# deevinandu/Distributed-Multi-Agent-SLAM-Swarm-Robotics-System

Measured on AMD Instinct MI355X. Metric: QuasarPackets/sec into 4096^2 grid, higher is better.
Workload: dtype f64

## Files before the change

### distributed-multi-agent-slam-swarm-robotics-system_amd/_lib.py

```python
import ctypes as C
import os
import subprocess

_HERE = os.path.dirname(os.path.abspath(__file__))
CSRC = os.path.join(_HERE, "csrc")
LIB_PATH = os.environ.get("QUASAR_SLAM_LIB") or os.path.join(CSRC, "libquasar_slam.so")
HEADER = os.path.join(os.path.dirname(_HERE), "include", "quasar_slam.h")

QS_CNT_NAMES = ("datagrams", "accepted", "rays", "cells", "hits", "closures", "landmarks", "rebases",
                "slam_windows", "slam_rounds", "slam_node_iters", "slam_misc_iters", "slam_cycles",
                "slam_realtime_100mhz", "slam_cyc_prepare", "slam_cyc_query", "slam_cyc_commit", "ekf_wrap_clamp", "edge_rays", "edge_overflow")
QS_FT_MAX_BOTS = 1024
QS_STAGE_NAMES = ("decode", "slam", "raycast", "ekf", "slam_chain", "rc_rays", "rc_sort", "rc_raster")
UINT64_MAX = (1 << 64) - 1
QS_PLAN_STATUS = ("ok", "no_start", "no_goal", "unreachable")


class QsPlanParams(C.Structure):
    _fields_ = [("clearance", C.c_int32), ("snap_radius", C.c_int32), ("lookahead", C.c_int32), ("reserved", C.c_int32)]


class QsGainParams(C.Structure):
    _fields_ = [("range", C.c_int32), ("bias", C.c_uint32), ("reserved", C.c_int32 * 2)]

# ... 141 lines not shown
    "qs_sense_ranges": (_i32, [_vp, _vp, _sz, _i32, _vp, _vp, _vp]),
    "qs_sense_ranges_device": (_i32, [_vp, _vp, _sz, _i32, _vp, _vp, _vp]),
    "qs_sense_sweeps": (_i32, [_vp, _vp, _vp, _vp, _vp, _sz, _vp, _vp, _sz]),
    "qs_sense_sweeps_device": (_i32, [_vp, _vp, _vp, _vp, _vp, _sz, _vp, _vp, _sz]),
    "qs_sense_packets": (_i32, [_vp, _vp, _vp, _vp, _vp, _vp, _sz, _vp, _vp]),
    "qs_sense_packets_device": (_i32, [_vp, _vp, _vp, _vp, _vp, _vp, _sz, _vp, _vp]),
    "qs_last_hits": (_i32, [_vp, _vp, _vp, _sz]),
    "qs_update_rays": (_i32, [_vp, _vp, _vp, _vp, _vp, _vp, _sz, _u64]),
    "qs_world_to_grid": (_i32, [_vp, _vp, _sz, _i32, _vp]),
    "qs_grid_i8": (_i32, [_vp, _vp]),
    "qs_grid_i8_device": (_i32, [_vp, _vp]),
    "qs_grid_counts": (_i32, [_vp, _vp, _vp]),
    "qs_grid_logodds": (_i32, [_vp, _f32, _f32, _f32, _f32, _vp]),
    "qs_device_buffers": (_i32, [_vp, C.POINTER(_vp), C.POINTER(_sz), C.POINTER(_vp), C.POINTER(_sz)]),
    "qs_slam_sizes": (_i32, [_vp, _i32, C.POINTER(_i64), C.POINTER(_i64), C.POINTER(_i64)]),
    "qs_slam_closures": (_i32, [_vp, _i32, _vp, _vp, _sz]),
    "qs_slam_closure_agents": (_i32, [_vp, _i32, _vp, _sz]),
    "qs_slam_landmarks": (_i32, [_vp, _i32, _vp, _vp, _sz]),
    "qs_slam_add_poses": (_i32, [_vp, _vp, _vp, _vp, _vp, _sz, _vp, _vp]),
    "qs_drift": (_i32, [_vp, _i32, _vp]),
    "qs_zone": (_i32, [_vp, _i32, _vp, C.POINTER(_i32)]),
    "qs_zone_packet": (_i32, [_vp, _i32, _i32, _vp]),
    "qs_fuse": (_i32, [_vp, C.POINTER(_vp), _sz]),
    "qs_fuse_buffers": (_i32, [_vp, C.POINTER(_vp), C.POINTER(_vp), _sz]),
    "qs_fuse_buffers_range": (_i32, [_vp, C.POINTER(_vp), C.POINTER(_vp), _sz, _sz, _sz, _i32]),
    "qs_fused_counts": (_i32, [_vp, C.POINTER(_vp), C.POINTER(_sz)]),
    "qs_counts_source": (_i32, [_vp, _i32]),
    "qs_epoch_query": (_i32, [_vp, _u64, _sz, C.POINTER(_i32)]),
    "qs_mark_fused": (_i32, [_vp]),
    "qs_dirty_tracking": (_i32, [_vp, _i32]),
    "qs_dirty_blocks": (_i32, [_vp, C.POINTER(_sz), C.POINTER(_sz)]),
    "qs_sparse_fuse_begin": (_i32, [_vp, _i32, _i32, C.POINTER(_vp), C.POINTER(_sz)]),
    "qs_sparse_fuse_plan": (_i32, [_vp, _vp, _vp, C.POINTER(_vp), C.POINTER(_sz)]),
    "qs_sparse_fuse_apply": (_i32, [_vp]),
    "qs_fused_counts_buffer": (_i32, [_vp, C.POINTER(_vp), C.POINTER(_sz)]),
    "qs_rccl_unique_id": (_i32, [_vp]),
    "qs_rccl_comm_init": (_i32, [_vp, _vp, _i32, _i32, C.POINTER(_vp)]),
    "qs_rccl_comm_destroy": (_i32, [_vp]),
    "qs_sparse_fuse_rccl": (_i32, [_vp, _vp, _i32, _i32, _vp]),
    "qs_grid_to_pcd": (_i32, [_vp, _vp, _i32, _i32, _f64, _f64, _f64, _vp, _sz, C.POINTER(_sz)]),
    "qs_rasterise": (_i32, [_vp, _vp, _sz, _f64, _vp, _vp, _vp]),
    "qs_icp": (_i32, [_vp, _vp, _sz, _vp, _sz, _f64, _i32, _f64, _f64, _vp, _vp, _vp, _vp]),
    "qs_nn_search": (_i32, [_vp, _vp, _sz, _vp, _sz, _f64, _i32, _vp, _vp, _vp]),
    "qs_diag_mfma_f64_rate": (_i32, [_vp, C.POINTER(_f64)]),
    "qs_diag_latencies": (_i32, [_vp, _vp]),
    "qs_set_chain_form": (_i32, [_vp, _i32]),
    "qs_chain_form": (_i32, [_vp]),
    "qs_set_chain_lean": (_i32, [_vp, _i32, _i64]),
    "qs_chain_lean": (_i32, [_vp]),
    "qs_set_chain_lookahead": (_i32, [_vp, _i32]),
    "qs_chain_lookahead": (_i32, [_vp]),
    "qs_set_chain_plan": (_i32, [_vp, _i32]),
    "qs_chain_plan": (_i32, [_vp]),
    "qs_voxel_downsample": (_i32, [_vp, _vp, _sz, _f64, _vp, _sz, C.POINTER(_sz)]),
    "qs_voxel_downsample_device": (_i32, [_vp, _vp, _sz, _f64, _vp, _sz, C.POINTER(_sz)]),
    "qs_merge_reset": (_i32, [_vp]),
    "qs_merge_params": (_i32, [_vp, _f64, _i32, _f64]),
    "qs_merge_grid": (_i32, [_vp, _vp, _i32, _i32, _f64, _f64, _f64, _vp]),
    "qs_merge_grid_device": (_i32, [_vp, _vp, _i32, _i32, _f64, _f64, _f64, _vp]),
    "qs_merge_map": (_i32, [_vp, _vp, _vp]),
    "qs_merge_cloud": (_i32, [_vp, _vp, _sz, C.POINTER(_sz)]),
    "qs_merge_global_map": (_i32, [_vp, _vp, _vp, _vp]),
    "qs_frontier_cells": (_i32, [_vp, _vp, _sz, C.POINTER(_sz)]),
    "qs_frontier_members": (_i32, [_vp, _vp, _sz, C.POINTER(_sz)]),
    "qs_frontier_clusters": (_i32, [_vp, _i32, _vp, _sz, C.POINTER(_sz)]),
    "qs_frontier_targets": (_i32, [_vp, _i32, _f64, _vp, _sz, _vp, _vp, _vp, _sz, C.POINTER(_sz), _vp]),
    "qs_traversable": (_i32, [_vp, _i32, _vp]),
    "qs_plan_field": (_i32, [_vp, _vp, _vp, _vp]),
    "qs_plan_paths": (_i32, [_vp, _vp, _vp, _vp, _sz, _vp, _vp, _vp, _vp, _vp, _sz, _vp, _vp]),
    "qs_frontier_targets_by_path": (_i32, [_vp, _i32, _f64, _vp, _vp, _sz, _vp, _vp, _vp, _vp, _vp, _vp, _vp, _sz,
                                           C.POINTER(_sz), _vp]),
    "qs_frontier_gain": (_i32, [_vp, _i32, _i32, _vp, _vp, _sz, C.POINTER(_sz)]),
    "qs_frontier_targets_by_gain": (_i32, [_vp, _i32, _f64, _vp, _vp, _vp, _sz, _vp, _vp, _vp, _vp, _vp, _vp, _vp, _sz,
                                           C.POINTER(_sz), _vp, _vp]),
    "qs_territories": (_i32, [_vp, _vp, _vp, _sz, _vp, _vp, _vp, _vp, _vp, _vp]),
    "qs_frontier_targets_by_territory": (_i32, [_vp, _i32, _vp, _vp, _sz, _vp, _vp, _vp, _vp, _vp, _vp, _vp, _vp, _vp, _vp, _sz,
                                                C.POINTER(_sz), _vp]),
    "qs_render_view": (_i32, [_vp, _vp, _vp, _sz, _vp, _sz, _vp]),
    "qs_render_view_device": (_i32, [_vp, _vp, _vp, _sz, _vp, _sz, _vp]),
    "qs_ekf_init": (_i32, [_vp, _i32, _f64, _vp]),
    "qs_ekf_step": (_i32, [_vp, _vp, _vp, _vp, _vp, _vp, _sz, _i32]),
    "qs_ekf_state": (_i32, [_vp, _i32, _vp, _vp]),
    "qs_counters": (_i32, [_vp, _vp]),
    "qs_checkpoint": (_i32, [_vp, _vp, _sz, C.POINTER(_sz)]),
    "qs_restore": (_i32, [_vp, _vp, _sz]),
    "qs_timing_enable": (_i32, [_vp, _i32]),
    "qs_stage_times": (_i32, [_vp, _vp, _vp, _i32]),
}


def load():
    global _lib
    if _lib is not None:
        return _lib
    if not os.path.exists(LIB_PATH):
        raise QuasarError(
            f"{LIB_PATH} not found: build it with __graft_entry__.build() (hipcc --offload-arch=gfx950). "
            "There is no CPU fallback for the mapper path.")
    L = C.CDLL(LIB_PATH)
    for name, (res, args) in SIGNATURES.items():
        fn = getattr(L, name)
        fn.restype = res
        fn.argtypes = args
    _lib = L
    return L

# ... 6 lines not shown
```

### distributed-multi-agent-slam-swarm-robotics-system_amd/csrc/qs_api.hip

```cpp
#include <math.h>
#include <algorithm>
#include <mutex>
#include <stdio.h>
#include <stdlib.h>
#include <string.h>

#include "qs_internal.h"
#include "raycast_common.h"

static thread_local std::string g_create_err;

int qs_fail(qs_ctx *c, int code, const char *what, hipError_t e)
{
    char buf[512];
    if (e != hipSuccess) snprintf(buf, sizeof buf, "%s: %s", what, hipGetErrorString(e));
    else snprintf(buf, sizeof buf, "%s", what);
    if (c) c->err = buf; else g_create_err = buf;
    return code;
}

extern "C" const char *qs_version(void) { return "quasar-slam-amd 0.1 (gfx950)"; }

extern "C" int qs_config_default(qs_config *cfg)
{
// ... 280 lines not shown
        HIPCHK(c, hipStreamCreateWithFlags(&c->stream, hipStreamNonBlocking));
        c->own_stream = true;
    }
    return QS_OK;
}

extern "C" int qs_set_chain_form(qs_ctx *c, int form)
{
    ARGCHK(c, c != nullptr);
    ARGCHK(c, form == QS_CHAIN_AUTO || form == QS_CHAIN_FREE || form == QS_CHAIN_WINDOW || form == QS_CHAIN_FREE_POSTING);
    c->chain_form = form;
    return QS_OK;
}

extern "C" int qs_chain_form(qs_ctx *c)
{
    if (!c) return QS_E_INVAL;
    return !c->chain_last_free ? QS_CHAIN_WINDOW : c->chain_last_posting ? QS_CHAIN_FREE_POSTING : QS_CHAIN_FREE;
}

extern "C" int qs_set_chain_lean(qs_ctx *c, int32_t mode, int64_t limit)
{
    ARGCHK(c, c != nullptr);
    ARGCHK(c, mode == QS_CHAIN_LEAN_AUTO || mode == QS_CHAIN_LEAN_OFF);
    c->chain_lean_mode = mode;
    c->chain_lean_limit = limit > 0 && limit < 0x7f7f7f7fll ? limit : 0x7f7f7f7fll;
    return QS_OK;
}

extern "C" int qs_chain_lean(qs_ctx *c)
{
    if (!c) return QS_E_INVAL;
    if (!c->chain_last_lean_asked) return 0;
    unsigned int refused = 0;
    HIPCHK(c, hipMemcpyAsync(&refused, c->d_flags.p + QS_FLAG_CHAIN_FULL, sizeof refused, hipMemcpyDeviceToHost, c->stream));
    HIPCHK(c, hipStreamSynchronize(c->stream));
    return refused != c->chain_lean_seq ? 1 : 0;
}

extern "C" int qs_set_chain_plan(qs_ctx *c, int32_t on)
{
    ARGCHK(c, c != nullptr);
    c->chain_plan = on != 0;
    return QS_OK;
}

extern "C" int qs_chain_plan(qs_ctx *c)
{
    if (!c) return QS_E_INVAL;
    if (!c->chain_last_plan) return 0;
    return qs_chain_lean(c);
}

extern "C" int qs_set_chain_lookahead(qs_ctx *c, int32_t on)
{
    ARGCHK(c, c != nullptr);
    c->chain_lookahead = on != 0;
    return QS_OK;
}

extern "C" int qs_chain_lookahead(qs_ctx *c)
{
    if (!c) return QS_E_INVAL;
    return c->chain_lookahead ? 1 : 0;
}

extern "C" int qs_sync(qs_ctx *c)
{
    ARGCHK(c, c != nullptr);
    HIPCHK(c, hipSetDevice(c->device));
    SYNCCHK(c);
    HIPCHK(c, hipStreamSynchronize(c->stream));
    return QS_OK;
}

extern "C" int qs_reset(qs_ctx *c)
{
    ARGCHK(c, c != nullptr);
    HIPCHK(c, hipSetDevice(c->device));
    return reset_state(c);
}

extern "C" int qs_set_bot_offset(qs_ctx *c, int32_t bot, double off_x)
{
    ARGCHK(c, c != nullptr);
    if (bot < 1 || bot > c->cfg.max_agent) return qs_fail(c, QS_E_RANGE, "qs_set_bot_offset: bot out of range");
    HIPCHK(c, hipSetDevice(c->device));
    HIPCHK(c, hipMemcpyAsync(c->d_offset.p + bot, &off_x, sizeof(double), hipMemcpyHostToDevice, c->stream));
    HIPCHK(c, hipStreamSynchronize(c->stream));
    return QS_OK;
}

extern "C" int qs_timing_enable(qs_ctx *c, int32_t enable)
{
    ARGCHK(c, c != nullptr);
    c->timing = enable != 0;
    return QS_OK;
}

extern "C" int qs_stage_times(qs_ctx *c, double ms[QS_STAGE_N], uint64_t launches[QS_STAGE_N], int32_t reset)
{
    ARGCHK(c, c != nullptr);
    HIPCHK(c, hipSetDevice(c->device));
    HIPCHK(c, hipStreamSynchronize(c->stream));
    for (auto &p : c->pending) {
        float t = 0.f;
// ... 676 lines not shown
```

### distributed-multi-agent-slam-swarm-robotics-system_amd/csrc/slam.hip

```cpp
#include "qs_internal.h"
#include <cstdlib>
#include <cstring>

#define LL_MAX 0x7fffffffffffffffll
#define IDX_BLOCK QS_SLAM_IDX_BLOCK
#define IDX_WAVES (IDX_BLOCK / QS_WAVE)

int qs_slam_blocks(size_t n) { return (int)((n + IDX_BLOCK - 1) / IDX_BLOCK); }

__global__ void __launch_bounds__(IDX_BLOCK)
qs_slam_count_kernel(size_t n, QsBatch b, QsSlamBatch sb, int bots_per_graph, int n_graphs)
{
    __shared__ unsigned int s_acc[QS_MAX_AGENT + 1], s_ev[QS_MAX_AGENT + 1];
    const int tid = threadIdx.x;
    for (int t = tid; t < n_graphs; t += IDX_BLOCK) { s_acc[t] = 0; s_ev[t] = 0; }
    __syncthreads();
    const size_t i = (size_t)blockIdx.x * IDX_BLOCK + tid;
    if (i < n && b.accept[i]) {
        const int g = ((int)b.agent[i] - 1) / bots_per_graph;
        atomicAdd(&s_acc[g], 1u);
        if (b.lm[i]) atomicAdd(&s_ev[g], 1u);
    }
    __syncthreads();
    for (int t = tid; t < n_graphs; t += IDX_BLOCK) {
        sb.blk_acc[(size_t)t * sb.n_blocks + blockIdx.x] = s_acc[t];
        sb.blk_ev[(size_t)t * sb.n_blocks + blockIdx.x] = s_ev[t];
    }
}

__global__ void __launch_bounds__(256)
qs_slam_blockscan_kernel(QsSlamBatch sb)
{
    __shared__ unsigned int s_a[256], s_e[256];
    const int g = blockIdx.x, tid = threadIdx.x;
    unsigned int *acc = sb.blk_acc + (size_t)g * sb.n_blocks, *ev = sb.blk_ev + (size_t)g * sb.n_blocks;
    const int per = (sb.n_blocks + 255) / 256;
    const int lo = min(tid * per, sb.n_blocks), hi = min(lo + per, sb.n_blocks);
    unsigned int a = 0, e = 0;
    for (int k = lo; k < hi; k++) { a += acc[k]; e += ev[k]; }
    s_a[tid] = a; s_e[tid] = e;
    __syncthreads();
    if (tid == 0) {
        unsigned int ra = 0, re = 0;
        for (int t = 0; t < 256; t++) { const unsigned int va = s_a[t], ve = s_e[t]; s_a[t] = ra; s_e[t] = re; ra += va; re += ve; }
        sb.acc_total[g] = ra;
        sb.ev_base[g + 1] = re;
    }
    __syncthreads();
    unsigned int ra = s_a[tid], re = s_e[tid];
    for (int k = lo; k < hi; k++) { const unsigned int va = acc[k], ve = ev[k]; acc[k] = ra; ev[k] = re; ra += va; re += ve; }
}

__global__ void qs_slam_prefix_kernel(QsSlamBatch sb, int n_graphs, int max_agent, const double *__restrict__ drift)
{
    if (threadIdx.x == 0) {
        unsigned int run = 0;
        sb.ev_base[0] = 0;
        for (int g = 0; g < n_graphs; g++) { run += sb.ev_base[g + 1]; sb.ev_base[g + 1] = run; }
    }
    if (threadIdx.x == 64) {
        unsigned int run = 0;
        for (int a = 0; a <= max_agent + 1; a++) { const unsigned int v = a <= max_agent ? sb.agent_ev[a] : 0; sb.agent_ev[a] = run; run += v; }
    }
    for (int t = threadIdx.x; t <= max_agent; t += blockDim.x) {
        sb.acl_cnt[t] = 0;
        sb.drift_start[2 * t] = drift[2 * t];
        sb.drift_start[2 * t + 1] = drift[2 * t + 1];
    }
}

__global__ void __launch_bounds__(IDX_BLOCK)
qs_slam_index_kernel(size_t n, QsBatch b, QsSlamBatch sb, const QsGraphDev *__restrict__ graphs,
                     int bots_per_graph, int n_graphs)
{
    extern __shared__ unsigned int s_w[];
    const int tid = threadIdx.x, lane = tid & 63, wave = tid >> 6;
    for (int t = tid; t < IDX_WAVES * n_graphs * 2; t += IDX_BLOCK) s_w[t] = 0;
    __syncthreads();
    const size_t i = (size_t)blockIdx.x * IDX_BLOCK + tid;
    const bool acc = i < n && b.accept[i];
    int g = -1, agent = 0, lmk = 0;
    if (acc) { agent = b.agent[i]; g = (agent - 1) / bots_per_graph; lmk = b.lm[i]; }
    unsigned int rank = 0, rank_ev = 0;
    unsigned long long remaining = __ballot(acc);
    while (remaining) {
        const int leader = __ffsll((long long)remaining) - 1;
        const int k = __shfl(g, leader);
        const unsigned long long grp = __ballot(acc && g == k);
        const unsigned long long egrp = __ballot(acc && g == k && lmk != 0);
        if (acc && g == k) {
            rank = __popcll(grp & ((1ull << lane) - 1));
            rank_ev = __popcll(egrp & ((1ull << lane) - 1));
            if (lane == leader) {
                s_w[(wave * n_graphs + k) * 2] = __popcll(grp);
                s_w[(wave * n_graphs + k) * 2 + 1] = __popcll(egrp);
            }
        }
        remaining &= ~grp;
    }
    __syncthreads();
    if (acc) {
        unsigned int off = 0, off_ev = 0;
        for (int w = 0; w < wave; w++) { off += s_w[(w * n_graphs + g) * 2]; off_ev += s_w[(w * n_graphs + g) * 2 + 1]; }
        const long long node = graphs[g].n_nodes + sb.blk_acc[(size_t)g * sb.n_blocks + blockIdx.x] + off + rank;
        sb.node[i] = node;
        if (lmk) {
            const size_t e = (size_t)sb.ev_base[g] + sb.blk_ev[(size_t)g * sb.n_blocks + blockIdx.x] + off_ev + rank_ev;
            sb.ev_node[e] = node;
            sb.ev_agent[e] = (unsigned char)(agent - 1 - g * bots_per_graph);
            sb.ev_type[e] = (unsigned char)lmk;
            sb.ev_px[e] = b.px[i];
            sb.ev_py[e] = b.py[i];
        }
    } else if (i < n) {
        sb.node[i] = -1;
    }
}

#define PLAN_BLOCK QS_SLAM_PLAN_BLOCK
#define PLAN_WAVES (PLAN_BLOCK / QS_WAVE)
int qs_slam_plan_blocks(size_t n) { return (int)((n + PLAN_BLOCK - 1) / PLAN_BLOCK); }

__device__ inline int plan_graph_of(const unsigned int *__restrict__ ev_base, int n_graphs, unsigned int e)
{
    int lo = 0, hi = n_graphs - 1;
    while (lo < hi) { const int mid = (lo + hi + 1) >> 1; if (ev_base[mid] <= e) lo = mid; else hi = mid - 1; }
    return lo;
}

__global__ void __launch_bounds__(PLAN_BLOCK)
qs_slam_plan_count_kernel(QsSlamBatch sb, int bots_per_graph, int n_graphs, int max_agent)
{
    __shared__ unsigned int s_cnt[QS_MAX_AGENT + 1];
    const int tid = threadIdx.x;
    const unsigned int n_ev = sb.ev_base[n_graphs], e = blockIdx.x * PLAN_BLOCK + tid;
    if (blockIdx.x * PLAN_BLOCK >= n_ev) return;
    for (int t = tid; t <= max_agent; t += PLAN_BLOCK) s_cnt[t] = 0;
    __syncthreads();
    if (e < n_ev) atomicAdd(&s_cnt[plan_graph_of(sb.ev_base, n_graphs, e) * bots_per_graph + 1 + sb.ev_agent[e]], 1u);
    __syncthreads();
    for (int t = tid; t <= max_agent; t += PLAN_BLOCK) sb.pl_blk[(size_t)t * sb.pl_blocks + blockIdx.x] = s_cnt[t];
}

__global__ void __launch_bounds__(256)
qs_slam_plan_scan_kernel(QsSlamBatch sb, int n_graphs)
{
    __shared__ unsigned int s_c[256];
    const int tid = threadIdx.x;
    const int used = (int)((sb.ev_base[n_graphs] + PLAN_BLOCK - 1) / PLAN_BLOCK);
    unsigned int *cnt = sb.pl_blk + (size_t)blockIdx.x * sb.pl_blocks;
    const int per = (used + 255) / 256;
    const int lo = min(tid * per, used), hi = min(lo + per, used);
    unsigned int c = 0;
    for (int k = lo; k < hi; k++) c += cnt[k];
    s_c[tid] = c;
    __syncthreads();
    for (int d = 1; d < 256; d <<= 1) {
        const unsigned int v = tid >= d ? s_c[tid - d] : 0u;
        __syncthreads();
        s_c[tid] += v;
        __syncthreads();
    }
    unsigned int run = s_c[tid] - c;
    for (int k = lo; k < hi; k++) { const unsigned int v = cnt[k]; cnt[k] = run; run += v; }
}

__global__ void __launch_bounds__(PLAN_BLOCK)
qs_slam_plan_scatter_kernel(QsSlamBatch sb, int bots_per_graph, int n_graphs, int max_agent)
{
    __shared__ unsigned int s_w[PLAN_WAVES][QS_MAX_AGENT + 1];
    const int tid = threadIdx.x, lane = tid & 63, wave = tid >> 6;
    const unsigned int n_ev = sb.ev_base[n_graphs], e = blockIdx.x * PLAN_BLOCK + tid;
    if (blockIdx.x * PLAN_BLOCK >= n_ev) return;
    for (int t = tid; t < PLAN_WAVES * (QS_MAX_AGENT + 1); t += PLAN_BLOCK) (&s_w[0][0])[t] = 0;
    __syncthreads();
    const bool have = e < n_ev;
    int g = 0, bot = -1;
    if (have) { g = plan_graph_of(sb.ev_base, n_graphs, e); bot = g * bots_per_graph + 1 + sb.ev_agent[e]; }
    unsigned int rank = 0;
    unsigned long long remaining = __ballot(have);
    while (remaining) {
        const int k = __shfl(bot, __ffsll((long long)remaining) - 1);
        const unsigned long long grp = __ballot(have && bot == k);
        if (have && bot == k) {
            rank = __popcll(grp & ((1ull << lane) - 1));
            if (rank == 0) s_w[wave][k] = __popcll(grp);
        }
        remaining &= ~grp;
    }
    __syncthreads();
    if (have && bot <= max_agent) {
        unsigned int off = sb.pl_blk[(size_t)bot * sb.pl_blocks + blockIdx.x] + rank;
        for (int w = 0; w < wave; w++) off += s_w[w][bot];
        QsPlanRec rec;
        rec.node = (int)sb.ev_node[e]; rec.r = e - sb.ev_base[g]; rec.type = sb.ev_type[e]; rec.skip = 0;
        rec.px = sb.ev_px[e]; rec.py = sb.ev_py[e];
        sb.pl_rec[sb.agent_ev[bot] + off] = rec;
    }
}

__device__ inline unsigned int plan_first_at_least(const QsPlanRec *pl, unsigned int from, unsigned int n_own, long long bound)
{
    unsigned int lo = from, hi = n_own, step = 1;
    while (lo < n_own) {
        const unsigned int p = step - 1 < n_own - 1 - lo ? lo + step - 1 : n_own - 1;
        if ((long long)pl[p].node >= bound) { hi = p; break; }
        lo = p + 1;
        if (step < (1u << 30)) step <<= 1;
    }
    while (lo < hi) { const unsigned int mid = lo + ((hi - lo) >> 1); if ((long long)pl[mid].node >= bound) hi = mid; else lo = mid + 1; }
    return lo;
}

__global__ void __launch_bounds__(256)
qs_slam_plan_skip_kernel(QsSlamBatch sb, int n_graphs, int max_agent, int min_between, const long long *__restrict__ last_closure)
{
    const unsigned int n_ev = sb.ev_base[n_graphs], s = blockIdx.x * 256 + threadIdx.x;
    if (s >= n_ev) return;
    int lo = 0, hi = max_agent;
    while (lo < hi) { const int mid = (lo + hi + 1) >> 1; if (sb.agent_ev[mid] <= s) lo = mid; else hi = mid - 1; }
    const int bot = lo;
    if (bot < 1) return;
    const unsigned int base = sb.agent_ev[bot], n_own = sb.agent_ev[bot + 1] - base, j = s - base;
    const QsPlanRec *const pl = sb.pl_rec + base;
    sb.pl_rec[base + j].skip = plan_first_at_least(pl, j + 1, n_own, (long long)pl[j].node + (long long)min_between);
    if (j == 0) sb.pl_first[bot] = plan_first_at_least(pl, 0, n_own, last_closure[bot] + (long long)min_between);
}

#define CH_WAVES 16
#define CH_PILE_NODES 64
#define CH_THREADS (CH_WAVES * QS_WAVE)
#define CH_INS (CH_WAVES - 1)
#define CH_FETCH (CH_WAVES - 2)
#define CH_AGW (CH_WAVES - 3)

__device__ inline void lds_barrier()
{
    __builtin_amdgcn_fence(__ATOMIC_RELEASE, "workgroup", "local");
    __builtin_amdgcn_s_barrier();
    __builtin_amdgcn_fence(__ATOMIC_ACQUIRE, "workgroup", "local");
}

__device__ inline int bucket_coord(double v, double b0, double inv_cell)
{
    const double f = floor((v - b0) * inv_cell);
    return (int)fmin(fmax(f, -1.0e9), 1.0e9);
}

__device__ inline long long rl64(long long v, int src_lane)
{
    int lo = (int)(v & 0xffffffffll), hi = (int)(v >> 32);
    lo = __builtin_amdgcn_readlane(lo, src_lane);
    hi = __builtin_amdgcn_readlane(hi, src_lane);
    return ((long long)hi << 32) | (unsigned int)lo;
}

__device__ inline unsigned int bucket_hash(int cx, int cy, unsigned int hmask)
{
    unsigned int h = ((unsigned int)cx * 0x9E3779B1u) ^ ((unsigned int)cy * 0x85EBCA77u);
    h ^= h >> 15;
    return h & hmask;
}
__device__ inline bool bucket_cell(double x, double y, int type, const QsBucketGeom &bg, int &cx, int &cy)
{
    cx = bucket_coord(x, bg.bx0, bg.inv_cell); cy = bucket_coord(y, bg.by0, bg.inv_cell);
    return type >= 1 && type <= QS_NTYPES;
}
__device__ inline long long bucket_key(int type, int cx, int cy, const QsBucketGeom &bg)
{
    return (long long)(type - 1) * ((long long)bg.hmask + 1) + bucket_hash(cx, cy, bg.hmask);
}


#define QS_GLOBAL __attribute__((address_space(1)))
typedef const QS_GLOBAL QsLmNode *QsNodeG;
typedef const QS_GLOBAL unsigned int *QsU32G;

__device__ inline void chain_insert_lanes(const QsGraphDev &G, bool inw, int rank, long long idx, long long kb, double x, double y,
                                          int type, int k, int lane, long long &n_lms, long long &n_misc, unsigned int &pool, bool &pile)
// ... 1212 lines not shown
    auto load = [&](long long e, double &x, double &y, long long &idx, int &type) {
        const bool in = e + lane < L.n;
        x = in ? L.x[e + lane] : 0.0; y = in ? L.y[e + lane] : 0.0;
        idx = in ? L.idx[e + lane] : LL_MAX; type = in ? (int)L.type[e + lane] : 0;
    };
    double x, y; long long idx; int type;
    load(0, x, y, idx, type);
    for (long long e = 0; e < L.n; e += QS_WAVE) {
        double xn, yn; long long idxn; int typen;
        load(e + QS_WAVE, xn, yn, idxn, typen);
        const int k = (int)(L.n - e < QS_WAVE ? L.n - e : QS_WAVE);
        const bool inw = lane < k;
        int cx, cy;
        const long long kb = (inw && bucket_cell(x, y, type, bg, cx, cy)) ? bucket_key(type, cx, cy, bg) : -1;
        chain_insert_lanes(G, inw, lane, idx, kb, x, y, type, k, lane, n_lms, n_misc, pool, pile);
        x = xn; y = yn; idx = idxn; type = typen;
    }
    if (lane == 0) {
        Gp->n_nodes = L.n_nodes; Gp->n_cls = L.n_cls;
        Gp->n_lms = n_lms; Gp->n_misc = n_misc; Gp->nodes_used = pool;
        if (pile) *pile_flag = 1u;
    }
}
hipError_t qs_launch_slam_rebuild_index(qs_ctx *c, const QsIndexLog *d_logs)
{
    if (c->n_graphs <= 0) return hipSuccess;
    hipLaunchKernelGGL(qs_slam_rebuild_index_kernel, dim3(c->n_graphs), dim3(QS_WAVE), 0, c->stream, c->d_graphs.p, c->bg, d_logs,
                       c->d_flags.p + QS_FLAG_PILE);
    return hipGetLastError();
}

hipError_t qs_launch_slam(qs_ctx *c, size_t n, bool raw_pose)
{
    if (n == 0) return hipSuccess;
    QsSlamBatch sb = c->sb;
    sb.n_blocks = qs_slam_blocks(n);
    const int G = c->n_graphs;
    hipLaunchKernelGGL(qs_slam_count_kernel, dim3(sb.n_blocks), dim3(IDX_BLOCK), 0, c->stream, n, c->b, sb,
                       c->bots_per_graph, G);
    hipLaunchKernelGGL(qs_slam_blockscan_kernel, dim3(G), dim3(256), 0, c->stream, sb);
    hipLaunchKernelGGL(qs_slam_prefix_kernel, dim3(1), dim3(256), 0, c->stream, sb, G, c->cfg.max_agent, c->d_drift.p);
    hipLaunchKernelGGL(qs_slam_index_kernel, dim3(sb.n_blocks), dim3(IDX_BLOCK), (size_t)IDX_WAVES * G * 2 * sizeof(unsigned int),
                       c->stream, n, c->b, sb, c->d_graphs.p, c->bots_per_graph, G);
    const bool one = c->bots_per_graph <= CH_AGW;
    const bool free_mode = c->chain_form != QS_CHAIN_WINDOW && !(c->chain_form == QS_CHAIN_AUTO && one && c->chain_windowed);
    const bool post = c->chain_form == QS_CHAIN_FREE_POSTING || (c->chain_form == QS_CHAIN_AUTO && c->chain_posting);
    const int sel = (c->pile_mode ? 4 : 0) | (c->bots_per_graph <= 5 ? 2 : 0) | (post ? 1 : 0);
    const bool lean_asked = free_mode && one && c->chain_lean_mode != QS_CHAIN_LEAN_OFF && !post && sel != 6;
    const bool plan = lean_asked && c->chain_plan && !raw_pose && !c->pile_mode;
    c->chain_last_plan = plan;
    if (plan) {
        sb.pl_blocks = qs_slam_plan_blocks(n);
        const int nbots = c->cfg.max_agent + 1;
        hipLaunchKernelGGL(qs_slam_plan_count_kernel, dim3(sb.pl_blocks), dim3(PLAN_BLOCK), 0, c->stream, sb, c->bots_per_graph, G, c->cfg.max_agent);
        hipLaunchKernelGGL(qs_slam_plan_scan_kernel, dim3(nbots), dim3(256), 0, c->stream, sb, G);
        hipLaunchKernelGGL(qs_slam_plan_scatter_kernel, dim3(sb.pl_blocks), dim3(PLAN_BLOCK), 0, c->stream, sb, c->bots_per_graph, G, c->cfg.max_agent);
        hipLaunchKernelGGL(qs_slam_plan_skip_kernel, dim3((unsigned int)((n + 255) / 256)), dim3(256), 0, c->stream, sb, G,
                           c->cfg.max_agent, c->cfg.min_poses_between, c->d_last_closure.p);
    } else {
        sb.pl_rec = nullptr;
    }
    StageTimer t_chain(c, QS_STAGE_SLAM_CHAIN);
#define CH_LAUNCH(ONE_, DENSE_) hipLaunchKernelGGL((qs_slam_chain_kernel<ONE_, DENSE_>), dim3(G), dim3(CH_THREADS), 0, c->stream, c->d_graphs.p, sb, c->bg, \
                           c->bots_per_graph, c->cfg.max_agent, c->win, c->cfg.min_poses_between, c->r2_threshold,                          \
                           c->cfg.closure_correction, c->d_drift.p, c->d_last_closure.p, c->d_counters.p, raw_pose ? 1 : 0, c->d_flags.p + QS_FLAG_PILE)
    c->chain_last_posting = false;
    c->chain_last_free = free_mode;
    c->chain_last_lean_asked = false;
#define FR_LAUNCH(DENSE_, WAVES_, POST_) hipLaunchKernelGGL((qs_slam_chain_free_kernel<DENSE_, WAVES_, POST_>), dim3(G), dim3(WAVES_ * QS_WAVE), 0, c->stream, c->d_graphs.p, sb, c->bg, \
                           c->bots_per_graph, c->cfg.max_agent, c->cfg.min_poses_between, c->r2_threshold,                                  \
                           c->cfg.closure_correction, c->d_drift.p, c->d_last_closure.p, c->d_counters.p, raw_pose ? 1 : 0, c->d_flags.p + QS_FLAG_PILE, \
                           c->chain_lean_mode == QS_CHAIN_LEAN_OFF ? 0ll : c->chain_lean_limit, c->chain_lean_seq,                          \
                           (unsigned int)((c->chain_lookahead ? QS_NODE_LOOKAHEAD : QS_NODE_CAP - 1) * sizeof(long long)))
#define DY_LAUNCH(DENSE_) hipLaunchKernelGGL((qs_slam_chain_dyn_kernel<DENSE_>), dim3(G), dim3(CH_THREADS), 0, c->stream, c->d_graphs.p, sb, c->bg, \
                           c->bots_per_graph, c->cfg.max_agent, c->cfg.min_poses_between, c->r2_threshold,                                  \
                           c->cfg.closure_correction, c->d_drift.p, c->d_last_closure.p, c->d_counters.p, raw_pose ? 1 : 0, c->d_flags.p + QS_FLAG_PILE)
    if (free_mode) {
        if (one) {
            c->chain_lean_seq++;
            c->chain_last_lean_asked = lean_asked;
            switch (sel) {
            case 0: FR_LAUNCH(false, 16, false); break;  case 1: FR_LAUNCH(false, 16, true); break;
            case 2: FR_LAUNCH(false, 8, false); break;   case 3: FR_LAUNCH(false, 8, true); break;
            case 4: FR_LAUNCH(true, 16, false); break;   case 5: FR_LAUNCH(true, 16, true); break;
            case 6: FR_LAUNCH(true, 8, false); break;    default: FR_LAUNCH(true, 8, true); break;
            }
            c->chain_last_posting = post;
        }
        else { if (c->pile_mode) DY_LAUNCH(true); else DY_LAUNCH(false); }
    }
#undef DY_LAUNCH
    else if (c->pile_mode) { if (one) CH_LAUNCH(true, true); else CH_LAUNCH(false, true); }
    else { if (one) CH_LAUNCH(true, false); else CH_LAUNCH(false, false); }
#undef FR_LAUNCH
#undef CH_LAUNCH
    t_chain.stop();
    if (raw_pose) return hipGetLastError();
    hipLaunchKernelGGL(qs_slam_pose_kernel, dim3((unsigned int)((n + 255) / 256)), dim3(256), 0, c->stream, n, c->b, sb);
    return hipGetLastError();
}
```

### distributed-multi-agent-slam-swarm-robotics-system_amd/mapper.py

```python
import ctypes as C
import os
import struct
import types
import zlib

import numpy as np

from . import _lib
from ._lib import QsConfig, QsMergeResult, QsViewParams, QS_MERGE_STATUS, QuasarError, UINT64_MAX, check
from . import protocol as P


def _ptr(a):
    return a.ctypes.data_as(C.c_void_p) if a is not None else None


def _dev_addr(a):
    return int(a.data_ptr()) if hasattr(a, "data_ptr") else int(a or 0)


CKPT_MAGIC = b"QSCK"
CKPT_VERSION = 1
CKPT_HEADER_FIXED = 144
CKPT_SECTIONS = {1: "scalars", 2: "bots", 3: "counters", 4: "graphs", 5: "block_ids", 6: "blocks", 7: "dirty"}
# ... 749 lines not shown
        dims = np.zeros(2, dtype=np.int32)
        origin = np.zeros(2, dtype=np.float64)
        self._chk(self._L.qs_rasterise(self._h, _ptr(xy), len(xy), res, _ptr(dims), _ptr(origin), None),
                  "qs_rasterise")
        if len(xy) == 0:
            return None, None
        grid = np.empty((int(dims[0]), int(dims[1])), dtype=np.int8)
        self._chk(self._L.qs_rasterise(self._h, _ptr(xy), len(xy), res, _ptr(dims), _ptr(origin), _ptr(grid)),
                  "qs_rasterise")
        return grid, origin

    def icp(self, src_xy, dst_xy, max_dist=1.0, max_iter=30, rel_fitness=1e-6, rel_rmse=1e-6):
        a = np.ascontiguousarray(src_xy, dtype=np.float64); b = np.ascontiguousarray(dst_xy, dtype=np.float64)
        T = np.zeros(9, dtype=np.float64)
        fit, rm, it = C.c_double(), C.c_double(), C.c_int32()
        self._chk(self._L.qs_icp(self._h, _ptr(a), len(a), _ptr(b), len(b), max_dist, max_iter, rel_fitness, rel_rmse,
                                 _ptr(T), C.byref(fit), C.byref(rm), C.byref(it)), "qs_icp")
        return T.reshape(3, 3), fit.value, rm.value, it.value

    def nn_search(self, src_xy, dst_xy, max_dist=1.0, mode=0):
        a = np.ascontiguousarray(src_xy, dtype=np.float64); b = np.ascontiguousarray(dst_xy, dtype=np.float64)
        corr = np.empty(len(a), dtype=np.int32); d2 = np.empty(len(a), dtype=np.float64)
        ms = np.zeros(2, dtype=np.float32)
        self._chk(self._L.qs_nn_search(self._h, _ptr(a), len(a), _ptr(b), len(b), max_dist, mode, _ptr(corr), _ptr(d2), _ptr(ms)),
                  "qs_nn_search")
        return corr, d2, (float(ms[0]), float(ms[1]))

    CHAIN_FORMS = {"auto": 0, "free": 1, "window": 2, "free_posting": 3}

    def set_chain_form(self, form):
        self._chk(self._L.qs_set_chain_form(self._h, self.CHAIN_FORMS[form]), "qs_set_chain_form")

    def chain_form(self):
        return {1: "free", 2: "window", 3: "free_posting"}[self._L.qs_chain_form(self._h)]

    def set_chain_lean(self, mode="auto", limit=0):
        self._chk(self._L.qs_set_chain_lean(self._h, {"auto": 0, "off": 1}[mode], int(limit)), "qs_set_chain_lean")

    def chain_lean(self):
        r = self._L.qs_chain_lean(self._h)
        if r < 0:
            self._chk(r, "qs_chain_lean")
        return bool(r)

    def set_chain_plan(self, on=True):
        self._chk(self._L.qs_set_chain_plan(self._h, 1 if on else 0), "qs_set_chain_plan")

    def chain_plan(self):
        r = self._L.qs_chain_plan(self._h)
        if r < 0:
            self._chk(r, "qs_chain_plan")
        return bool(r)

    def set_chain_lookahead(self, on=True):
        self._chk(self._L.qs_set_chain_lookahead(self._h, 1 if on else 0), "qs_set_chain_lookahead")

    def chain_lookahead(self):
        r = self._L.qs_chain_lookahead(self._h)
        if r < 0:
            self._chk(r, "qs_chain_lookahead")
        return bool(r)

    def mfma_f64_rate(self):
        v = C.c_double()
        self._chk(self._L.qs_diag_mfma_f64_rate(self._h, C.byref(v)), "qs_diag_mfma_f64_rate")
        return v.value

    def diag_latencies(self):
        out = np.zeros(9, dtype=np.float64)
        self._chk(self._L.qs_diag_latencies(self._h, _ptr(out)), "qs_diag_latencies")
        names = ("l2_load", "l1_load", "lds_read", "fma_f64", "dpp_step", "readlane_step", "barrier_16_waves", "barrier_5_waves", "clock_mhz")
        return dict(zip(names, (float(v) for v in out)))

    def voxel_downsample(self, xy, voxel):
        a = np.ascontiguousarray(xy, dtype=np.float64)
        n = C.c_size_t()
        self._chk(self._L.qs_voxel_downsample(self._h, _ptr(a), len(a), voxel, None, 0, C.byref(n)), "qs_voxel_downsample")
        out = np.zeros((n.value, 2), dtype=np.float64)
        if n.value:
            self._chk(self._L.qs_voxel_downsample(self._h, _ptr(a), len(a), voxel, _ptr(out), n.value, C.byref(n)),
                      "qs_voxel_downsample")
        return out

    def voxel_downsample_device(self, d_xy, n, voxel, d_out=0, cap=0):
        k = C.c_size_t()
        self._chk(self._L.qs_voxel_downsample_device(self._h, C.c_void_p(_dev_addr(d_xy)), int(n), voxel,
                                                     C.c_void_p(_dev_addr(d_out)), int(cap), C.byref(k)), "qs_voxel_downsample_device")
        return k.value

    def merge_reset(self):
        self._chk(self._L.qs_merge_reset(self._h), "qs_merge_reset")

    def merge_params(self, icp_threshold=1.0, icp_iterations=30, min_fitness=0.6):
        self._chk(self._L.qs_merge_params(self._h, icp_threshold, icp_iterations, min_fitness), "qs_merge_params")

    @staticmethod
    def _merge_result(r):
        return {"status": QS_MERGE_STATUS[r.status], "iterations": int(r.iterations), "n_local": int(r.n_local),
                "n_global": int(r.n_global), "fitness": float(r.fitness), "rmse": float(r.rmse),
                "T": np.array(r.T, dtype=np.float64).reshape(3, 3)}

    def merge_grid(self, grid, res, ox, oy):
        r = QsMergeResult()
        if hasattr(grid, "data_ptr"):
            if not (grid.is_cuda and grid.is_contiguous() and grid.dim() == 2 and grid.element_size() == 1):
                raise ValueError("merge_grid: a device grid is a contiguous 2-D int8 tensor on the GPU")
# ... 510 lines not shown
```

### include/quasar_slam.h

```cpp
#ifndef QUASAR_SLAM_H
#define QUASAR_SLAM_H

#include <stddef.h>
#include <stdint.h>

#ifdef __cplusplus
extern "C" {
#endif

#define QS_OK 0
#define QS_E_INVAL (-1)
#define QS_E_HIP (-2)
#define QS_E_NOMEM (-3)
#define QS_E_RANGE (-4)
#define QS_E_NODEV (-5)
#define QS_E_STATE (-6)

#define QS_PACKET_SIZE 42
#define QS_PACKET_SIZE_V1 41
#define QS_ZONE_SIZE 20

typedef struct qs_ctx qs_ctx;

typedef struct qs_config {
// ... 133 lines not shown
                      const uint8_t *landmark, size_t n, uint8_t *closed, double *corr2);
int qs_drift(qs_ctx *ctx, int32_t bot, double out[2]);

int qs_zone(qs_ctx *ctx, int32_t bot, double out[4], int32_t *valid);
int qs_zone_packet(qs_ctx *ctx, int32_t bot, int32_t online, uint8_t out[QS_ZONE_SIZE]);

int qs_fuse(qs_ctx *dst, qs_ctx *const *srcs, size_t n);
int qs_fuse_buffers(qs_ctx *dst, const void *const *stamps_dev, const void *const *counts_dev,
                    size_t n);
int qs_fuse_buffers_range(qs_ctx *dst, const void *const *stamps_dev, const void *const *counts_dev,
                          size_t n, size_t cell_offset, size_t n_cells, int32_t counts_into_fused);
int qs_fused_counts(qs_ctx *ctx, void **fused_dev, size_t *bytes);
int qs_counts_source(qs_ctx *ctx, int32_t fused);
int qs_epoch_query(qs_ctx *ctx, uint64_t seq0, size_t n, int32_t *would_rebase);
int qs_mark_fused(qs_ctx *ctx);
#define QS_DIRTY_BLOCK_W 16
#define QS_DIRTY_BLOCK_H 4
#define QS_SPARSE_MAX_WORLD 64
int qs_dirty_tracking(qs_ctx *ctx, int32_t enable);
int qs_dirty_blocks(qs_ctx *ctx, size_t *n_blocks, size_t *block_cells);
int qs_sparse_fuse_begin(qs_ctx *ctx, int32_t world, int32_t rank, void **bitmaps_dev, size_t *bitmap_bytes);
int qs_sparse_fuse_plan(qs_ctx *ctx, uint32_t *n_blocks , size_t *offsets ,
                        void **payload_dev, size_t *block_bytes);
int qs_sparse_fuse_apply(qs_ctx *ctx);
#define QS_RCCL_ID_BYTES 128
int qs_rccl_unique_id(uint8_t out[QS_RCCL_ID_BYTES]);
int qs_rccl_comm_init(qs_ctx *ctx, const uint8_t id[QS_RCCL_ID_BYTES], int32_t world, int32_t rank, void **comm);
int qs_rccl_comm_destroy(void *comm);
int qs_sparse_fuse_rccl(qs_ctx *ctx, void *comm, int32_t world, int32_t rank, uint64_t stats[4]);
int qs_fused_counts_buffer(qs_ctx *ctx, void **fused_dev, size_t *bytes);
int qs_grid_to_pcd(qs_ctx *ctx, const int8_t *grid, int32_t h, int32_t w, double res,
                   double ox, double oy, double *xy, size_t cap, size_t *n_out);
int qs_rasterise(qs_ctx *ctx, const double *xy, size_t n, double res, int32_t dims[2],
                 double origin[2], int8_t *grid);

int qs_icp(qs_ctx *ctx, const double *src_xy, size_t n_src, const double *dst_xy, size_t n_dst,
           double max_dist, int32_t max_iter, double rel_fitness, double rel_rmse, double T[9],
           double *fitness, double *rmse, int32_t *iters);
int qs_nn_search(qs_ctx *ctx, const double *src_xy, size_t n_src, const double *dst_xy, size_t n_dst,
                 double max_dist, int32_t mode, int32_t *corr, double *d2, float ms[2]);
#define QS_CHAIN_AUTO 0
#define QS_CHAIN_FREE 1
#define QS_CHAIN_WINDOW 2
#define QS_CHAIN_FREE_POSTING 3
int qs_set_chain_form(qs_ctx *ctx, int form);
int qs_chain_form(qs_ctx *ctx);
#define QS_CHAIN_LEAN_AUTO 0
#define QS_CHAIN_LEAN_OFF 1
int qs_set_chain_lean(qs_ctx *ctx, int32_t mode, int64_t limit);
int qs_chain_lean(qs_ctx *ctx);

int qs_set_chain_plan(qs_ctx *ctx, int32_t on);
int qs_chain_plan(qs_ctx *ctx);

int qs_set_chain_lookahead(qs_ctx *ctx, int32_t on);
int qs_chain_lookahead(qs_ctx *ctx);

int qs_diag_mfma_f64_rate(qs_ctx *ctx, double *tflops);
#define QS_DIAG_LAT_N 9
int qs_diag_latencies(qs_ctx *ctx, double out[QS_DIAG_LAT_N]);
int qs_voxel_downsample(qs_ctx *ctx, const double *xy, size_t n, double voxel, double *out_xy,
                        size_t cap, size_t *n_out);

int qs_voxel_downsample_device(qs_ctx *ctx, const double *d_xy, size_t n, double voxel, double *d_out_xy,
                               size_t cap, size_t *n_out);

enum { QS_MERGE_EMPTY = 0, QS_MERGE_ADOPTED = 1, QS_MERGE_MERGED = 2, QS_MERGE_REJECTED = 3 };
typedef struct qs_merge_result {
    int32_t status, iterations;
    uint64_t n_local, n_global;
    double fitness, rmse, T[9];
} qs_merge_result;
int qs_merge_reset(qs_ctx *ctx);
int qs_merge_params(qs_ctx *ctx, double icp_threshold, int32_t icp_iterations, double min_fitness);
int qs_merge_grid(qs_ctx *ctx, const int8_t *grid, int32_t h, int32_t w, double res, double ox, double oy,
                  qs_merge_result *out);
int qs_merge_grid_device(qs_ctx *ctx, const int8_t *d_grid, int32_t h, int32_t w, double res, double ox, double oy,
                         qs_merge_result *out);
int qs_merge_map(qs_ctx *ctx, qs_ctx *src, qs_merge_result *out);
int qs_merge_cloud(qs_ctx *ctx, double *xy, size_t cap, size_t *n_out);
int qs_merge_global_map(qs_ctx *ctx, int32_t dims[2], double origin[2], int8_t *grid);

int qs_frontier_cells(qs_ctx *ctx, int32_t *xy, size_t cap, size_t *n_out);
int qs_frontier_clusters(qs_ctx *ctx, int32_t min_cluster, int64_t *stats5, size_t cap, size_t *n_out);

int qs_frontier_members(qs_ctx *ctx, int32_t *xy_root, size_t cap, size_t *n_out);

#define QS_FT_MAX_BOTS 1024
int qs_frontier_targets(qs_ctx *ctx, int32_t min_cluster, double separation,
                        const double *bot_xy, size_t n_bots, int64_t *target_idx, double *target_xy,
                        double *centroids_xy, size_t cap, size_t *n_centroids, uint64_t stats[4]);

#define QS_PLAN_OK 0
#define QS_PLAN_NO_START 1
#define QS_PLAN_NO_GOAL 2
#define QS_PLAN_UNREACHABLE 3
#define QS_PLAN_ORTHO 5
#define QS_PLAN_DIAG 7
#define QS_PLAN_MAX_CLEARANCE 16
#define QS_PLAN_MAX_SNAP 64
#define QS_PLAN_MAX_LOOKAHEAD 65536
#define QS_PLAN_WS_CAP ((size_t)2 << 30)
typedef struct qs_plan_params { int32_t clearance, snap_radius, lookahead, reserved; } qs_plan_params;
int qs_traversable(qs_ctx *ctx, int32_t clearance, uint8_t *mask_host);
int qs_plan_field(qs_ctx *ctx, const qs_plan_params *params, const double goal_xy[2], uint32_t *field_host);
int qs_plan_paths(qs_ctx *ctx, const qs_plan_params *params, const double *start_xy, const double *goal_xy, size_t n,
// ... 107 lines not shown
```

Before: 102.2 million.

## Fold plan skip computation into scatter kernel with shared-memory halo search

```diff
diff --git a/distributed-multi-agent-slam-swarm-robotics-system_amd/_lib.py b/distributed-multi-agent-slam-swarm-robotics-system_amd/_lib.py
--- a/distributed-multi-agent-slam-swarm-robotics-system_amd/_lib.py
+++ b/distributed-multi-agent-slam-swarm-robotics-system_amd/_lib.py
@@ -217,6 +217,7 @@
     "qs_chain_lookahead": (_i32, [_vp]),
     "qs_set_chain_plan": (_i32, [_vp, _i32]),
     "qs_chain_plan": (_i32, [_vp]),
+    "qs_chain_plan_read": (_i32, [_vp, _i32, _vp, _vp, _vp, _sz, C.POINTER(_sz), C.POINTER(C.c_uint32)]),
     "qs_voxel_downsample": (_i32, [_vp, _vp, _sz, _f64, _vp, _sz, C.POINTER(_sz)]),
     "qs_voxel_downsample_device": (_i32, [_vp, _vp, _sz, _f64, _vp, _sz, C.POINTER(_sz)]),
     "qs_merge_reset": (_i32, [_vp]),
diff --git a/distributed-multi-agent-slam-swarm-robotics-system_amd/csrc/qs_api.hip b/distributed-multi-agent-slam-swarm-robotics-system_amd/csrc/qs_api.hip
--- a/distributed-multi-agent-slam-swarm-robotics-system_amd/csrc/qs_api.hip
+++ b/distributed-multi-agent-slam-swarm-robotics-system_amd/csrc/qs_api.hip
@@ -356,6 +356,28 @@
     return qs_chain_lean(c);
 }
 
+extern "C" int qs_chain_plan_read(qs_ctx *c, int32_t bot, int32_t *node, uint32_t *r, uint32_t *skip, size_t cap, size_t *n_own,
+                                  uint32_t *first)
+{
+    ARGCHK(c, c != nullptr && n_own && first);
+    ARGCHK(c, (node && r && skip) || (!node && !r && !skip));
+    if (bot < 1 || bot > c->cfg.max_agent) return qs_fail(c, QS_E_RANGE, "qs_chain_plan_read: bot out of range");
+    if (!c->chain_last_plan) return qs_fail(c, QS_E_STATE, "qs_chain_plan_read: the last ingest had no plan");
+    HIPCHK(c, hipSetDevice(c->device));
+    unsigned int range[2] = {0, 0}, f = 0;
+    HIPCHK(c, hipMemcpyAsync(range, c->sb.agent_ev + bot, sizeof range, hipMemcpyDeviceToHost, c->stream));
+    HIPCHK(c, hipMemcpyAsync(&f, c->sb.pl_first + bot, sizeof f, hipMemcpyDeviceToHost, c->stream));
+    HIPCHK(c, hipStreamSynchronize(c->stream));
+    const size_t n = range[1] - range[0];
+    *n_own = n; *first = f;
+    if (!node) return QS_OK;
+    if (n > cap) return qs_fail(c, QS_E_RANGE, "qs_chain_plan_read: capacity too small");
+    std::vector<QsPlanRec> rec(n);
+    if (n) HIPCHK(c, hipMemcpy(rec.data(), c->sb.pl_rec + range[0], n * sizeof(QsPlanRec), hipMemcpyDeviceToHost));
+    for (size_t i = 0; i < n; i++) { node[i] = rec[i].node; r[i] = rec[i].r; skip[i] = rec[i].skip; }
+    return QS_OK;
+}
+
 extern "C" int qs_set_chain_lookahead(qs_ctx *c, int32_t on)
 {
     ARGCHK(c, c != nullptr);
diff --git a/distributed-multi-agent-slam-swarm-robotics-system_amd/csrc/slam.hip b/distributed-multi-agent-slam-swarm-robotics-system_amd/csrc/slam.hip
--- a/distributed-multi-agent-slam-swarm-robotics-system_amd/csrc/slam.hip
+++ b/distributed-multi-agent-slam-swarm-robotics-system_amd/csrc/slam.hip
@@ -64,6 +64,7 @@
     }
     for (int t = threadIdx.x; t <= max_agent; t += blockDim.x) {
         sb.acl_cnt[t] = 0;
+        sb.pl_first[t] = 0;
         sb.drift_start[2 * t] = drift[2 * t];
         sb.drift_start[2 * t + 1] = drift[2 * t + 1];
     }
@@ -129,17 +130,25 @@
 }
 
 __global__ void __launch_bounds__(PLAN_BLOCK)
-qs_slam_plan_count_kernel(QsSlamBatch sb, int bots_per_graph, int n_graphs, int max_agent)
-{
-    __shared__ unsigned int s_cnt[QS_MAX_AGENT + 1];
+qs_slam_plan_count_kernel(QsSlamBatch sb, int bots_per_graph, int n_graphs, int max_agent, int min_between,
+                          const long long *__restrict__ last_closure)
+{
+    __shared__ unsigned int s_cnt[QS_MAX_AGENT + 1], s_cool[QS_MAX_AGENT + 1];
     const int tid = threadIdx.x;
     const unsigned int n_ev = sb.ev_base[n_graphs], e = blockIdx.x * PLAN_BLOCK + tid;
     if (blockIdx.x * PLAN_BLOCK >= n_ev) return;
-    for (int t = tid; t <= max_agent; t += PLAN_BLOCK) s_cnt[t] = 0;
+    for (int t = tid; t <= max_agent; t += PLAN_BLOCK) { s_cnt[t] = 0; s_cool[t] = 0; }
     __syncthreads();
-    if (e < n_ev) atomicAdd(&s_cnt[plan_graph_of(sb.ev_base, n_graphs, e) * bots_per_graph + 1 + sb.ev_agent[e]], 1u);
+    if (e < n_ev) {
+        const int bot = plan_graph_of(sb.ev_base, n_graphs, e) * bots_per_graph + 1 + sb.ev_agent[e];
+        atomicAdd(&s_cnt[bot], 1u);
+        if (bot <= max_agent && sb.ev_node[e] < last_closure[bot] + (long long)min_between) atomicAdd(&s_cool[bot], 1u);
+    }
     __syncthreads();
-    for (int t = tid; t <= max_agent; t += PLAN_BLOCK) sb.pl_blk[(size_t)t * sb.pl_blocks + blockIdx.x] = s_cnt[t];
+    for (int t = tid; t <= max_agent; t += PLAN_BLOCK) {
+        sb.pl_blk[(size_t)t * sb.pl_blocks + blockIdx.x] = s_cnt[t];
+        if (s_cool[t]) atomicAdd(&sb.pl_first[t], s_cool[t]);
+    }
 }
 
 __global__ void __launch_bounds__(256)
@@ -165,18 +174,23 @@
     for (int k = lo; k < hi; k++) { const unsigned int v = cnt[k]; cnt[k] = run; run += v; }
 }
 
+#define PLAN_HALO 256
 __global__ void __launch_bounds__(PLAN_BLOCK)
-qs_slam_plan_scatter_kernel(QsSlamBatch sb, int bots_per_graph, int n_graphs, int max_agent)
+qs_slam_plan_scatter_kernel(QsSlamBatch sb, int bots_per_graph, int n_graphs, int max_agent, int min_between, int window)
 {
     __shared__ unsigned int s_w[PLAN_WAVES][QS_MAX_AGENT + 1];
+    __shared__ long long s_node[PLAN_BLOCK + PLAN_HALO];
+    __shared__ unsigned char s_agent[PLAN_BLOCK + PLAN_HALO];
     const int tid = threadIdx.x, lane = tid & 63, wave = tid >> 6;
-    const unsigned int n_ev = sb.ev_base[n_graphs], e = blockIdx.x * PLAN_BLOCK + tid;
-    if (blockIdx.x * PLAN_BLOCK >= n_ev) return;
+    const unsigned int n_ev = sb.ev_base[n_graphs], e0 = blockIdx.x * PLAN_BLOCK, e = e0 + tid;
+    if (e0 >= n_ev) return;
     for (int t = tid; t < PLAN_WAVES * (QS_MAX_AGENT + 1); t += PLAN_BLOCK) (&s_w[0][0])[t] = 0;
+    for (int t = tid; t < PLAN_BLOCK + (window ? PLAN_HALO : 0); t += PLAN_BLOCK)
+        if (e0 + t < n_ev) { s_node[t] = sb.ev_node[e0 + t]; s_agent[t] = sb.ev_agent[e0 + t]; }
     __syncthreads();
     const bool have = e < n_ev;
     int g = 0, bot = -1;
-    if (have) { g = plan_graph_of(sb.ev_base, n_graphs, e); bot = g * bots_per_graph + 1 + sb.ev_agent[e]; }
+    if (have) { g = plan_graph_of(sb.ev_base, n_graphs, e); bot = g * bots_per_graph + 1 + s_agent[tid]; }
     unsigned int rank = 0;
     unsigned long long remaining = __ballot(have);
     while (remaining) {
@@ -192,8 +206,18 @@
     if (have && bot <= max_agent) {
         unsigned int off = sb.pl_blk[(size_t)bot * sb.pl_blocks + blockIdx.x] + rank;
         for (int w = 0; w < wave; w++) off += s_w[w][bot];
+        unsigned int skip = 0;
+        if (window) {
+            const long long bound = s_node[tid] + (long long)min_between;
+            const unsigned int end = min(sb.ev_base[g + 1], e + (unsigned int)window);
+            int lo = tid + 1, hi = (int)(end - e0);
+            while (lo < hi) { const int mid = (lo + hi) >> 1; if (s_node[mid] >= bound) hi = mid; else lo = mid + 1; }
+            const unsigned char own = s_agent[tid];
+            skip = off + 1;
+            for (int q = tid + 1; q < lo; q++) skip += s_agent[q] == own;
+        }
         QsPlanRec rec;
-        rec.node = (int)sb.ev_node[e]; rec.r = e - sb.ev_base[g]; rec.type = sb.ev_type[e]; rec.skip = 0;
+        rec.node = (int)s_node[tid]; rec.r = e - sb.ev_base[g]; rec.type = sb.ev_type[e]; rec.skip = skip;
         rec.px = sb.ev_px[e]; rec.py = sb.ev_py[e];
         sb.pl_rec[sb.agent_ev[bot] + off] = rec;
     }
@@ -213,7 +237,7 @@
 }
 
 __global__ void __launch_bounds__(256)
-qs_slam_plan_skip_kernel(QsSlamBatch sb, int n_graphs, int max_agent, int min_between, const long long *__restrict__ last_closure)
+qs_slam_plan_skip_kernel(QsSlamBatch sb, int n_graphs, int max_agent, int min_between)
 {
     const unsigned int n_ev = sb.ev_base[n_graphs], s = blockIdx.x * 256 + threadIdx.x;
     if (s >= n_ev) return;
@@ -224,7 +248,6 @@
     const unsigned int base = sb.agent_ev[bot], n_own = sb.agent_ev[bot + 1] - base, j = s - base;
     const QsPlanRec *const pl = sb.pl_rec + base;
     sb.pl_rec[base + j].skip = plan_first_at_least(pl, j + 1, n_own, (long long)pl[j].node + (long long)min_between);
-    if (j == 0) sb.pl_first[bot] = plan_first_at_least(pl, 0, n_own, last_closure[bot] + (long long)min_between);
 }
 
 #define CH_WAVES 16
@@ -1543,11 +1566,15 @@
     if (plan) {
         sb.pl_blocks = qs_slam_plan_blocks(n);
         const int nbots = c->cfg.max_agent + 1;
-        hipLaunchKernelGGL(qs_slam_plan_count_kernel, dim3(sb.pl_blocks), dim3(PLAN_BLOCK), 0, c->stream, sb, c->bots_per_graph, G, c->cfg.max_agent);
+        const int mb = c->cfg.min_poses_between, window = mb > PLAN_HALO ? 0 : mb > 1 ? mb : 1;
+        hipLaunchKernelGGL(qs_slam_plan_count_kernel, dim3(sb.pl_blocks), dim3(PLAN_BLOCK), 0, c->stream, sb, c->bots_per_graph, G, c->cfg.max_agent,
+                           mb, c->d_last_closure.p);
         hipLaunchKernelGGL(qs_slam_plan_scan_kernel, dim3(nbots), dim3(256), 0, c->stream, sb, G);
-        hipLaunchKernelGGL(qs_slam_plan_scatter_kernel, dim3(sb.pl_blocks), dim3(PLAN_BLOCK), 0, c->stream, sb, c->bots_per_graph, G, c->cfg.max_agent);
-        hipLaunchKernelGGL(qs_slam_plan_skip_kernel, dim3((unsigned int)((n + 255) / 256)), dim3(256), 0, c->stream, sb, G,
-                           c->cfg.max_agent, c->cfg.min_poses_between, c->d_last_closure.p);
+        hipLaunchKernelGGL(qs_slam_plan_scatter_kernel, dim3(sb.pl_blocks), dim3(PLAN_BLOCK), 0, c->stream, sb, c->bots_per_graph, G, c->cfg.max_agent,
+                           mb, window);
+        if (!window)
+            hipLaunchKernelGGL(qs_slam_plan_skip_kernel, dim3((unsigned int)((n + 255) / 256)), dim3(256), 0, c->stream, sb, G,
+                               c->cfg.max_agent, mb);
     } else {
         sb.pl_rec = nullptr;
     }
diff --git a/distributed-multi-agent-slam-swarm-robotics-system_amd/mapper.py b/distributed-multi-agent-slam-swarm-robotics-system_amd/mapper.py
--- a/distributed-multi-agent-slam-swarm-robotics-system_amd/mapper.py
+++ b/distributed-multi-agent-slam-swarm-robotics-system_amd/mapper.py
@@ -825,6 +825,15 @@
             self._chk(r, "qs_chain_plan")
         return bool(r)
 
+    def chain_plan_read(self, bot):
+        n, first = C.c_size_t(0), C.c_uint32(0)
+        self._chk(self._L.qs_chain_plan_read(self._h, bot, None, None, None, 0, C.byref(n), C.byref(first)), "qs_chain_plan_read")
+        node = np.empty(n.value, dtype=np.int32); r = np.empty(n.value, dtype=np.uint32); skip = np.empty(n.value, dtype=np.uint32)
+        if n.value:
+            self._chk(self._L.qs_chain_plan_read(self._h, bot, _ptr(node), _ptr(r), _ptr(skip), n.value, C.byref(n), C.byref(first)),
+                      "qs_chain_plan_read")
+        return {"node": node, "r": r, "skip": skip, "first": int(first.value)}
+
     def set_chain_lookahead(self, on=True):
         self._chk(self._L.qs_set_chain_lookahead(self._h, 1 if on else 0), "qs_set_chain_lookahead")
 
diff --git a/include/quasar_slam.h b/include/quasar_slam.h
--- a/include/quasar_slam.h
+++ b/include/quasar_slam.h
@@ -209,6 +209,8 @@
 
 int qs_set_chain_plan(qs_ctx *ctx, int32_t on);
 int qs_chain_plan(qs_ctx *ctx);
+int qs_chain_plan_read(qs_ctx *ctx, int32_t bot, int32_t *node, uint32_t *r, uint32_t *skip, size_t cap, size_t *n_own,
+                       uint32_t *first);
 
 int qs_set_chain_lookahead(qs_ctx *ctx, int32_t on);
 int qs_chain_lookahead(qs_ctx *ctx);
```

Measured after the change: 104.1 million (median of 6 runs). +1.8%, better.
